# lbcb-sci/herro

Hardware: AMD Instinct MI355X
Metric: 4096-bp windows corrected/sec at batch=128 (higher is better)
Workload: dtype f16; 1 GPU; synthetic windows, 4096 bp, 32 overlaps each, batch=128, 1xMI355X per rank (BASELINE configs[2]); batch=128, window=4096, overlaps=32, batches_per_launch_group=32, streams_per_gpu=2, distinct_windows_cycled=16384, precision=5, total_windows=165760, strong_leg_windows=0

## Files before the change

herro_amd/csrc/pileup.hip:

```cpp
#include <hip/hip_runtime.h>
#include <stdint.h>

#include <cstdio>
#include <cstdlib>
#include <mutex>
#include <set>
#include <type_traits>

#include "job_dev.h"
#include "pileup_core.h"

namespace herro {

namespace {

constexpr uint32_t NONE = 0xffffffffu;
constexpr uint32_t RF_LEFT = 0x80000000u;
constexpr uint32_t ROWCAP = HERRO_TILE;
constexpr uint32_t SCAP = 128;
constexpr uint32_t QEVCAP = 2048;

template <int NT>
__device__ __forceinline__ uint32_t blk_scan(uint32_t v, uint32_t* total, uint32_t* s_wave ) {
  const int lane = threadIdx.x & 63, wave = threadIdx.x >> 6;
// ... 484 lines not shown
  PROF_MARK(J, 1, 2);
  const bool in_lds = n <= RKCAP;
  if (in_lds)
    for (uint32_t i = tid; i < n; i += NT) { s_acc[i] = J.ow_acc[wd.ow_begin + i]; s_keep[i] = J.ow_keep[wd.ow_begin + i]; }
  __syncthreads();
  if (tid < 32 && tid < n && ((keepmask >> tid) & 1u) && s_ns) {
    const uint32_t cls = ocol[wd.ow_begin + tid].w, nm = (s_nm2[tid & 15u] >> (tid & 16u)) & 0xffffu, ns = s_ns;
    if (nm) atomicAdd(&J.nd[2 * (uint64_t)cls], nm);
    if (ns - nm) atomicAdd(&J.nd[2 * (uint64_t)cls + 1], ns - nm);
  }
  auto rank_all = [&](auto lds) {
    constexpr bool LDS = decltype(lds)::value;
    for (uint32_t i = tid; i < n; i += NT) {
      const uint32_t oi = wd.ow_begin + i;
      const uint32_t ki = LDS ? (uint32_t)s_keep[i] : (uint32_t)J.ow_keep[oi];
      if (!ki) continue;
      const float ai = LDS ? s_acc[i] : J.ow_acc[oi];
      uint32_t rank = 0;
      for (uint32_t j = 0; j < n; j++) {
        const uint32_t kj = LDS ? (uint32_t)s_keep[j] : (uint32_t)J.ow_keep[wd.ow_begin + j];
        const float aj = LDS ? s_acc[j] : J.ow_acc[wd.ow_begin + j];
        if (kj && (aj > ai || (aj == ai && j < i))) rank++;
      }
      J.slot_ow[wd.ow_begin + rank] = oi;
    }
  };
  if (in_lds) rank_all(std::true_type{}); else rank_all(std::false_type{});
  if (tid == 0) J.win_nkept[w] = n_kept;
  PROF_MARK(J, 1, 3);
}

constexpr int LY_NT = 256;
constexpr uint32_t TCAP = 2 * LY_NT;
#define MI(p) ((p) + ((p) >> 4))
__host__ __device__ inline size_t layout_lds(uint32_t W) { return (size_t)(W + 1 + ((W + 1) >> 4) + 1) * 4; }

template <bool TILES>
__global__ __launch_bounds__(LY_NT) void k_layout(JobDev J) {
  extern __shared__ __attribute__((aligned(16))) uint32_t ly_smem[];
  uint32_t* s_mi = ly_smem;
  __shared__ double s_score[SCAP];
  __shared__ uint32_t s_sel[32], s_nev[32], s_evoff[32], s_wave[LY_NT / 64], s_maxne, s_nrun;
  __shared__ uint32_t s_tcnt[TCAP], s_toff[TCAP];
  const uint32_t w = blockIdx.x, tid = threadIdx.x;
  PROF_BEGIN(J);
  const WinDesc wd = J.win[w];
  const uint32_t n_kept = J.win_nkept[w];
  const uint32_t win_len = wd.win_len;
  if (tid < 32) s_sel[tid] = NONE;
  if (tid == 0) { s_maxne = 0; s_nrun = 0; }
  if constexpr (TILES) for (uint32_t t = tid; t < TCAP; t += LY_NT) s_tcnt[t] = 0;
  for (uint32_t p = tid; p <= win_len; p += LY_NT) s_mi[MI(p)] = 0;
  __syncthreads();
  PROF_MARK(J, 2, 5);
  {
    auto score_of = [&](uint32_t k) -> double {
      const uint32_t cls = J.ocol[J.slot_ow[wd.ow_begin + k]].w;
      const uint32_t nn = J.nd[2 * (uint64_t)cls], dd = J.nd[2 * (uint64_t)cls + 1];
      const uint32_t tot = nn + dd;
      if (!tot) return 0.0;
      const double lg = tot < J.ln_table_n ? J.ln_table[tot] : log((double)tot + 1.0);
      return __dmul_rn(__ddiv_rn((double)nn, (double)tot), lg);
    };
    const bool cached = n_kept <= SCAP;
    if (cached) {
      for (uint32_t k = tid; k < n_kept; k += LY_NT) s_score[k] = score_of(k);
      __syncthreads();
      PROF_MARK(J, 2, 6);
    }
    for (uint32_t k = tid; k < n_kept; k += LY_NT) {
      const uint32_t o = J.slot_ow[wd.ow_begin + k];
      const uint32_t qid = J.ow[o].qid;
      const double sk = cached ? s_score[k] : score_of(k);
      uint32_t rank = 0;
      if (cached) {
        uint32_t i = 0;
        for (; i + 8 <= n_kept; i += 8) {
          double sv[8];
#pragma unroll
          for (int u = 0; u < 8; u++) sv[u] = s_score[i + u];
#pragma unroll
          for (int u = 0; u < 8; u++) if (sv[u] > sk || (sv[u] == sk && i + u < k)) rank++;
        }
        for (; i < n_kept; i++) {
          const double si = s_score[i];
          if (si > sk || (si == sk && i < k)) rank++;
        }
      } else {
        for (uint32_t i = 0; i < n_kept; i++) {
          const double si = score_of(i);
          if (si > sk || (si == sk && i < k)) rank++;
        }
      }
      J.rank_qid[wd.ow_begin + rank] = qid;
      if (rank < 30u) s_sel[rank + 1] = o;
    }
    __syncthreads();
  }
  PROF_MARK(J, 2, 0);
  if (tid < 32) {
    CTab t;
    t.off = 0; t.t_total = 0; t.tokc = (uint32_t)TOK_GAP_F << 8; t.ow = NONE; t.n_ev = 0; t.ev_off = 0; t.sbase = 0; t.sdir = 1;
    t.qual_off = 0; t.q_woff = 0;
    if (tid == 0) {
      t.t_total = win_len;
      t.q_woff = J.read_word_off[wd.rid];
      t.qual_off = J.read_qual_off[wd.rid];
    } else if (s_sel[tid] != NONE) {
      const uint32_t o = s_sel[tid];
      const OwDesc& d = J.ow[o];
      t.off = (int32_t)(d.tstart - d.wtstart);
      t.t_total = J.ow_ttotal[o];
      t.tokc = d.strand ? (5u | ((uint32_t)TOK_GAP_R << 8)) : ((uint32_t)TOK_GAP_F << 8);
      t.ow = o;
      t.n_ev = J.ins_cnt[o];
      t.ev_off = d.scr_off;
      t.sbase = d.strand ? (int32_t)(d.qbeg + d.qlen - 1u) : (int32_t)d.qbeg;
      t.sdir = d.strand ? -1 : 1;
      t.qual_off = d.q_qual_off;
      t.q_woff = d.q_woff;
    }
    const uint32_t nev = tid == 0 ? 0u : t.n_ev;
    const uint32_t inc = wscan_incl(nev);
    const uint32_t tot = (uint32_t)__builtin_amdgcn_readlane((int)inc, 31);
    if (tid == 0) {
      t.ev_off = (uint32_t)wd.ev_off;
      t.n_ev = tot;
    }
    J.ctab[(uint64_t)w * 32 + tid] = t;
    J.sel_ow[(uint64_t)w * 32 + tid] = s_sel[tid];
    s_nev[tid] = nev;
    s_evoff[tid] = tid == 0 ? 0u : t.ev_off;
    if (tid == 0) s_evoff[0] = t.ev_off;
    atomicMax(&s_maxne, nev);
  }
  __syncthreads();
  PROF_MARK(J, 2, 1);
  const uint32_t lc = tid >> 3, sub = tid & 7u;
  const uint32_t ne = s_nev[lc];
  const uint64_t eo = s_evoff[lc], wbase = s_evoff[0];
  const uint32_t nbatch = (s_maxne + 63u) / 64u;
  uint4 v[8];
  uint32_t hx[8];
  auto load = [&](uint32_t b) {
#pragma unroll
    for (int k = 0; k < 8; k++) {
      const uint32_t i = b * 64u + sub + 8u * k;
      v[k] = ne ? J.iev[eo + min(i, ne - 1u)] : make_uint4(0, 0, 0, 0);
      if constexpr (TILES) hx[k] = ne ? J.iev[eo + min(i + 1u, ne - 1u)].x : 0u; else hx[k] = 0u;
    }
  };
  for (uint32_t b = 0; b < nbatch; b++) {
    load(b);
#pragma unroll
    for (int k = 0; k < 8; k++) {
      const uint32_t i = b * 64u + sub + 8u * k;
      if (i < ne) {
        const uint32_t p = v[k].x & 0xffffu;
        if (p < win_len) atomicMax(&s_mi[MI(p)], v[k].w);
      }
    }
  }
  __syncthreads();
  PROF_MARK(J, 2, 2);
  {
    const uint32_t ch = (win_len + LY_NT - 1) / LY_NT;
    const uint32_t p0 = min(tid * ch, win_len), p1 = min(p0 + ch, win_len);
    uint32_t local = 0;
    for (uint32_t p = p0; p < p1; p++) local += 1u + s_mi[MI(p)];
    uint32_t Lf;
    uint32_t r = blk_scan<LY_NT>(local, &Lf, s_wave);
    const uint32_t tile0 = (uint32_t)wd.col_off;
    for (uint32_t p = p0; p < p1; p++) {
      const uint32_t rn = r + 1u + s_mi[MI(p)];
      s_mi[MI(p)] = r;
      const uint32_t i = (rn - 1u) / ROWCAP;
      if (i * ROWCAP >= r) J.chdr2[tile0 + i] = make_uint2(p, r == i * ROWCAP ? 1u : 0u);
      r = rn;
    }
    if (tid == 0) { s_mi[MI(win_len)] = Lf; J.win_Lf[w] = Lf; }
  }
  __syncthreads();
  PROF_MARK(J, 2, 3);
  for (uint32_t p = tid; p <= win_len; p += LY_NT) J.row_of_pos2[wd.pos_off + p] = s_mi[MI(p)];
  const uint32_t tile0 = (uint32_t)wd.col_off, n_t = (s_mi[MI(win_len)] + ROWCAP - 1) / ROWCAP;
  auto each_run = [&](uint32_t b, auto&& fn) {
    if (nbatch > 1) load(b);
#pragma unroll
    for (int k = 0; k < 8; k++) {
      const uint32_t i = b * 64u + sub + 8u * k;
      if (i >= ne) continue;
      const uint32_t p = v[k].x & 0xffffu, len = v[k].x >> 16;
      if (p >= win_len) continue;
      const uint32_t rp = s_mi[MI(p)], room = s_mi[MI(p + 1)] - rp - 1u;
      uint32_t hide = 0;
      if (i + 1 < ne && (hx[k] & 0xffffu) == p) {
        hide = hx[k] >> 16;
        for (uint32_t e2 = i + 2; e2 < ne; e2++) {
          const uint32_t x3 = J.iev[eo + e2].x;
          if ((x3 & 0xffffu) != p) break;
          hide = max(hide, x3 >> 16);
        }
      }
      const uint32_t lenr = min(len, room);
      if (hide >= lenr) continue;
      fn(v[k], hide, (rp + 1u + hide) / ROWCAP, (rp + lenr) / ROWCAP);
    }
  };
  if constexpr (!TILES) {
    (void)n_t; (void)tile0; (void)wbase; (void)each_run;
  } else {
  for (uint32_t b = 0; b < nbatch; b++)
    each_run(b, [&](const uint4&, uint32_t, uint32_t t_lo, uint32_t t_hi) {
      for (uint32_t t = t_lo; t <= t_hi && t < TCAP; t++) atomicAdd(&s_tcnt[t], 1u);
    });
  __syncthreads();
  {
    uint32_t tot;
    const uint32_t c0 = s_tcnt[2 * tid], c1 = s_tcnt[2 * tid + 1];
    const uint32_t ex = blk_scan<LY_NT>(c0 + c1, &tot, s_wave);
    s_toff[2 * tid] = ex;
    s_toff[2 * tid + 1] = ex + c0;
    if (2 * tid < n_t) J.tile_ev[tile0 + 2 * tid] = make_uint2(ex, c0);
    if (2 * tid + 1 < n_t) J.tile_ev[tile0 + 2 * tid + 1] = make_uint2(ex + c0, c1);
  }
  __syncthreads();
  for (uint32_t b = 0; b < nbatch; b++)
    each_run(b, [&](const uint4& e, uint32_t hide, uint32_t t_lo, uint32_t t_hi) {
      for (uint32_t t = t_lo; t <= t_hi && t < TCAP; t++)
        J.tev[wbase + atomicAdd(&s_toff[t], 1u)] = make_uint4(e.x, e.y, e.z, lc | (hide << 8) | (t << 16));
    });
  }
  PROF_MARK(J, 2, 4);
}

constexpr int TK_NT = 256;
constexpr uint32_t WPAD = 36;

__device__ __forceinline__ uint32_t dpp_quad_add(uint32_t v) {
  v += (uint32_t)__builtin_amdgcn_mov_dpp((int)v, 0xB1, 0xf, 0xf, true);
  v += (uint32_t)__builtin_amdgcn_mov_dpp((int)v, 0x4E, 0xf, 0xf, true);
  return v;
}
__device__ __forceinline__ uint32_t dpp_quad_lane0(uint32_t v) {
  return (uint32_t)__builtin_amdgcn_mov_dpp((int)v, 0x00, 0xf, 0xf, true);
}

__global__ __launch_bounds__(TK_NT, 4) void k_tokens(JobDev J, uint32_t aux) {
  __shared__ __attribute__((aligned(16))) CTab s_ct[32];
  __shared__ __attribute__((aligned(16))) uint16_t s_rowinfo[ROWCAP];
  __shared__ uint32_t s_adj[ROWCAP];
  __shared__ uint32_t s_pl[HERRO_ROWS * 3 * WPAD];
  __shared__ uint32_t s_rop[ROWCAP + 4];
  __shared__ uint32_t s_supbits[ROWCAP / 32];
  const uint32_t tile = blockIdx.x, tid = threadIdx.x, nw = J.nw;
  PROF_BEGIN(J);
  const uint32_t w = J.tile_win[tile], r0 = J.tile_r0[tile];
  const uint32_t Lf = J.win_Lf[w];
  if (r0 >= Lf) return;
  const WinDesc wd = J.win[w];
  const uint2 ch0 = J.chdr2[tile];
  const bool last = r0 + ROWCAP >= Lf;
  const uint2 ch1 = J.chdr2[last ? tile : tile + 1];
  const uint2 tev_h = J.tile_ev[tile];
  if (tid < 32) s_ct[tid] = J.ctab[(uint64_t)w * 32 + tid];
// ... 227 lines not shown
  PROF_MARK(J, 3, 6);
}

__global__ __launch_bounds__(64) void k_supgather(JobDev J) {
  const uint32_t w = blockIdx.x, lane = threadIdx.x;
  const WinDesc wd = J.win[w];
  const uint32_t Lf = J.win_Lf[w], tile0 = (uint32_t)wd.col_off;
  const uint32_t nch = (Lf + ROWCAP - 1) / ROWCAP;
  uint32_t dst = 0;
  for (uint32_t c0 = 0; c0 < nch; c0 += 64) {
    const uint32_t i = c0 + lane;
    const uint32_t cn = i < nch ? J.tile_nsup[tile0 + i] : 0u;
    const uint32_t inc = wscan_incl(cn);
    const uint32_t my_dst = dst + inc - cn;
    for (uint32_t j = 0; j < 64 && c0 + j < nch; j++) {
      const uint32_t cnt_j = (uint32_t)__builtin_amdgcn_readlane((int)cn, (int)j), dst_j = (uint32_t)__builtin_amdgcn_readlane((int)my_dst, (int)j);
      const uint32_t src = (c0 + j) * ROWCAP;
      if (src == dst_j) continue;
      for (uint32_t k = lane; k < cnt_j; k += 64) {
        const uint32_t a = J.sup_row[wd.row_off + src + k], b = J.sup_pi[wd.row_off + src + k];
        J.sup_row[wd.row_off + dst_j + k] = a;
        J.sup_pi[wd.row_off + dst_j + k] = b;
      }
    }
    dst += wlast(inc);
  }
  if (lane == 0) J.win_nsup[w] = dst;
}

#ifndef HERRO_RW_ICAP
#define HERRO_RW_ICAP 2048
#endif
constexpr uint32_t RW_ICAP = HERRO_RW_ICAP;
#define RI(p) ((p) + ((p) >> 5))
__host__ __device__ inline size_t rows_lds(uint32_t W) { return (size_t)(W + 2 + ((W + 2) >> 5) + 1) * 4; }

constexpr uint32_t RW_SUPCAP = 256;
template <int SP>
__device__ __forceinline__ void rf_slot(const JobDev& J, const CTab* __restrict__ s_ct, const WinDesc& wd, uint32_t Lf, uint32_t half, uint32_t c,
                                        uint32_t srow, uint32_t pj, uint32_t nr, bool have_nr, uint4* __restrict__ out);

template <int NW>
__global__ __launch_bounds__(2 * NW) void k_rows(JobDev J) {
  constexpr int NT = 2 * NW;
  extern __shared__ __attribute__((aligned(16))) uint32_t rw_smem[];
  uint32_t* s_rop = rw_smem;
  uint32_t* s_mrg = rw_smem + rows_lds(J.window_size) / 4;
  __shared__ __attribute__((aligned(16))) CTab s_ct[32];
  __shared__ uint32_t s_adj[RW_ICAP];
  __shared__ __attribute__((aligned(16))) uint8_t s_iv[RW_ICAP];
  __shared__ uint32_t s_rfbase;
  __shared__ uint32_t s_sup[3][RW_SUPCAP];
  __shared__ uint32_t s_wave[NT / 64];
  const uint32_t w = blockIdx.x, tid = threadIdx.x, nw = J.nw;
  const uint32_t half = tid >= (uint32_t)NW ? 1u : 0u, lt = tid - half * NW;
  PROF_BEGIN(J);
  const WinDesc wd = J.win[w];
  const uint32_t Lf = J.win_Lf[w], win_len = wd.win_len;
  const uint32_t tile0 = (uint32_t)wd.col_off;
  {
    constexpr int RL = 17;
    uint32_t rv[RL];
    const uint32_t* __restrict__ rop = J.row_of_pos2 + wd.pos_off;
#pragma unroll
    for (int u = 0; u < RL; u++) rv[u] = rop[min(tid + (uint32_t)u * NT, win_len)];
    if (tid < 32) s_ct[tid] = J.ctab[(uint64_t)w * 32 + tid];
#pragma unroll
    for (int u = 0; u < RL; u++) {
      const uint32_t p = tid + (uint32_t)u * NT;
      if (p <= win_len) s_rop[RI(p)] = rv[u];
    }
  }
  __syncthreads();
  PROF_MARK(J, 6, 0);
  const bool active = lt < nw;
  const uint32_t widx = min(lt, nw - 1u);
  const int32_t P = (int32_t)(widx << 5);
  const uint32_t vm = active ? mask_range(0, (int32_t)win_len - P) : 0u;
  const uint64_t pmax = J.read_n_words + 1;
  const uint32_t tlo = glb_bits(J.read_p0, s_ct[0].q_woff, pmax, (int32_t)wd.tstart + P) & vm;
  const uint32_t thi = glb_bits(J.read_p1, s_ct[0].q_woff, pmax, (int32_t)wd.tstart + P) & vm;
  uint32_t c0[5], c1[5];
  uint32_t nin[5];
  const uint32_t tsym[4] = {vm & ~tlo & ~thi, tlo & ~thi, thi & ~tlo, tlo & thi};
#pragma unroll
  for (int q = 0; q < 4; q++) { c0[q] = half ? 0u : tsym[q]; c1[q] = 0; }
  c0[4] = 0; c1[4] = 0;
  nin[0] = half ? 0u : vm; nin[1] = 0; nin[2] = 0; nin[3] = 0; nin[4] = 0;
  auto sat_add = [&](int q, uint32_t x) { sat2_add(c0[q], c1[q], x); };
  {
    constexpr int UB = 15;
    const uint32_t cb = 1u + UB * half;
    uint32_t M[UB], L[UB], H[UB];
#pragma unroll
    for (int u = 0; u < UB; u++) {
      const uint32_t o = s_ct[cb + u].ow;
      const PlaneRec g = J.cw[(o != NONE ? (uint64_t)o : 0ull) * nw + widx];
      M[u] = g.m; L[u] = g.lo; H[u] = g.hi;
    }
    PROF_MARK(J, 6, 10);
#pragma unroll
    for (int u = 0; u < UB; u++) {
      const CTab& h = s_ct[cb + u];
      const uint32_t tt = h.ow != NONE ? h.t_total : 0u;
      const uint32_t inr = mask_range(h.off - P, h.off + (int32_t)tt - P) & vm;
      const uint32_t Mi = M[u] & inr, Li = L[u] & Mi, Hi = H[u] & Mi;
      sat_add(0, Mi & ~Li & ~Hi);
      sat_add(1, Li & ~Hi);
      sat_add(2, Hi & ~Li);
      sat_add(3, Li & Hi);
      sat_add(4, inr & ~Mi);
      uint32_t x = inr;
#pragma unroll
      for (int b = 0; b < 5; b++) { const uint32_t cy = nin[b] & x; nin[b] ^= x; x = cy; }
    }
  }
  if (half) {
#pragma unroll
    for (int q = 0; q < 5; q++) { s_mrg[(q) * NW + lt] = c0[q]; s_mrg[(5 + q) * NW + lt] = c1[q]; s_mrg[(10 + q) * NW + lt] = nin[q]; }
  }
  __syncthreads();
  if (!half) {
#pragma unroll
    for (int q = 0; q < 5; q++) sat2_merge(c0[q], c1[q], s_mrg[q * NW + lt], s_mrg[(5 + q) * NW + lt]);
    uint32_t cy = 0;
#pragma unroll
    for (int b = 0; b < 5; b++) {
      const uint32_t x = nin[b], y = s_mrg[(10 + b) * NW + lt];
      nin[b] = x ^ y ^ cy;
      cy = (x & y) | (cy & (x ^ y));
    }
  }
  const bool lane0 = !half && active;
  constexpr uint32_t IP_ROWS = (RW_ICAP * 2 + NW * 4 - 1) / (NW * 4);
  static_assert(IP_ROWS + 7 <= 15, "s_mrg holds the insertion rows' positions, five cover planes and two words per lane");
  uint16_t* s_ip = reinterpret_cast<uint16_t*>(s_mrg);
  uint32_t* s_nin = s_mrg + IP_ROWS * NW;
  uint32_t* s_insup = s_nin + 5 * NW;
  uint32_t* s_nisup = s_insup + NW;
  if (!half) {
#pragma unroll
    for (int b = 0; b < 5; b++) s_nin[b * NW + lt] = nin[b];
    s_insup[lt] = 0;
    s_nisup[lt] = 0;
  }
  PROF_MARK(J, 6, 1);
  const RowVotes rvt = base_row_votes(c0, c1, tsym, vm);
  const uint32_t supb = lane0 ? rvt.sup : 0u, V0 = rvt.v0, V1 = rvt.v1, V2 = rvt.v2;
  uint32_t insmask = 0;
  if (lane0) {
    uint32_t rprev = s_rop[RI((uint32_t)P)];
#pragma unroll 4
    for (uint32_t k = 0; k < 32; k++) {
      const uint32_t p = (uint32_t)P + k;
      const uint32_t rn = s_rop[RI(min(p + 1u, win_len))];
      if (p < win_len && rn - rprev > 1u) insmask |= 1u << k;
      rprev = rn;
    }
    uint32_t* __restrict__ vp = J.vpl + (uint64_t)w * 4 * nw + lt;
    vp[0] = V0; vp[nw] = V1; vp[2 * nw] = V2; vp[3 * nw] = insmask;
  }
  PROF_MARK(J, 6, 2);
  const uint32_t n_irows = Lf - win_len;
  uint32_t n_isup = 0, insup = 0;
  for (uint32_t ch0 = 0; ch0 < n_irows; ch0 += RW_ICAP) {
    if (ch0) __syncthreads();
    for (uint32_t i = tid; i < min(RW_ICAP, n_irows - ch0); i += NT) s_adj[i] = 0;
    __syncthreads();
    PROF_MARK(J, 6, 7);
    constexpr uint32_t TPC = NT / 32;
    constexpr int EU = 6;
    const uint32_t c = tid / TPC, sub = tid % TPC;
    const uint32_t ne = (c >= 1u && s_ct[c].ow != NONE) ? s_ct[c].n_ev : 0u;
    const uint4* __restrict__ iev = J.iev + s_ct[c].ev_off;
    for (uint32_t i0 = sub; i0 < ne; i0 += EU * TPC) {
      uint4 ve[EU];
      uint32_t nx[EU];
#pragma unroll
      for (int u = 0; u < EU; u++) {
        const uint32_t i = i0 + u * TPC;
        ve[u] = iev[min(i, ne - 1u)];
        nx[u] = iev[min(i + 1u, ne - 1u)].x;
      }
#pragma unroll
      for (int u = 0; u < EU; u++) {
        const uint32_t i = i0 + u * TPC;
        if (i >= ne) continue;
        const uint32_t p = ve[u].x & 0xffffu, len = ve[u].x >> 16;
        if (p >= win_len) continue;
        const uint32_t rp = s_rop[RI(p)], room = s_rop[RI(p + 1)] - rp - 1u;
        uint32_t hide = 0;
        if (i + 1u < ne && (nx[u] & 0xffffu) == p) {
          hide = nx[u] >> 16;
          for (uint32_t e2 = i + 2u; e2 < ne; e2++) {
            const uint32_t x3 = iev[e2].x;
            if ((x3 & 0xffffu) != p) break;
            hide = max(hide, x3 >> 16);
          }
        }
        const bool inr = (uint32_t)((int32_t)p - s_ct[c].off) < s_ct[c].t_total;
        for (uint32_t k = hide; k < len && k < room; k++) {
          const uint32_t ir = rp + k - p - ch0;
          if (ir >= RW_ICAP) continue;
          uint32_t code;
          if (k < 16u) code = ((ve[u].z >> k) & 1u) | (((ve[u].z >> (16u + k)) & 1u) << 1);
          else {
            const int32_t si = s_ct[c].sbase + s_ct[c].sdir * (int32_t)(ve[u].y + k);
            const uint64_t wi = min(s_ct[c].q_woff + ((uint32_t)si >> 5), pmax);
            code = ((J.read_p0[wi] >> ((uint32_t)si & 31u)) & 1u) | (((J.read_p1[wi] >> ((uint32_t)si & 31u)) & 1u) << 1);
            if (s_ct[c].sdir < 0) code ^= 3u;
          }
          atomicAdd(&s_adj[ir], (1u << (5u * code)) + (inr ? 1u << 20 : 0u));
          s_ip[ir] = (uint16_t)p;
        }
      }
    }
    __syncthreads();
    PROF_MARK(J, 6, 8);
    for (uint32_t i = tid; i < min(RW_ICAP, n_irows - ch0); i += NT) {
      const uint32_t adj = s_adj[i];
      uint32_t cover = 0, p = 0;
      if (adj) {
        p = s_ip[i];
        const uint32_t pw = p >> 5, pb = p & 31u;
        cover = ((s_nin[pw] >> pb) & 1u) | (((s_nin[NW + pw] >> pb) & 1u) << 1) | (((s_nin[2 * NW + pw] >> pb) & 1u) << 2) |
                (((s_nin[3 * NW + pw] >> pb) & 1u) << 3) | (((s_nin[4 * NW + pw] >> pb) & 1u) << 4);
      }
      const uint32_t c5[5] = {adj & 31u, (adj >> 5) & 31u, (adj >> 10) & 31u, (adj >> 15) & 31u, cover - (adj >> 20)};
      uint32_t ns = 0;
#pragma unroll
      for (int q = 0; q < 5; q++) ns += c5[q] >= 3u ? 1u : 0u;
      s_iv[i] = (uint8_t)(vote5(c5, 4u) | ((ns >= 2u ? 1u : 0u) << 7));
      if (ns >= 2u) { atomicOr(&s_insup[p >> 5], 1u << (p & 31u)); atomicAdd(&s_nisup[p >> 5], 1u); }
    }
    __syncthreads();
    PROF_MARK(J, 6, 9);
    if (lane0) { insup = s_insup[lt]; n_isup = s_nisup[lt]; }
    {
      const uint32_t nb = min(RW_ICAP, n_irows - ch0);
      uint32_t* __restrict__ dst = reinterpret_cast<uint32_t*>(J.cons_tmp + wd.row_off + ch0);
      for (uint32_t i = tid; i * 4u < nb; i += NT) dst[i] = reinterpret_cast<const uint32_t*>(s_iv)[i];
    }
  }
// ... 695 lines not shown
  KT_BEGIN(tm, "rf_quals", st);
  if (rf && 2 * half + 1 <= 8) {
    if (half <= 2u) hipLaunchKernelGGL(k_rfq<5>, dim3(J.n_win), dim3(RQ_NT), 0, st, J, half, sup_off, rf, cap, (lean ? 1u : 0u) | (left_only ? 2u : 0u));
    else hipLaunchKernelGGL(k_rfq<8>, dim3(J.n_win), dim3(RQ_NT), 0, st, J, half, sup_off, rf, cap, (lean ? 1u : 0u) | (left_only ? 2u : 0u));
    KT_END(tm, st);
    return;
  }
  pileup_opt_in_lds(reinterpret_cast<const void*>(k_quals<false>), 96 * 1024);
  hipLaunchKernelGGL(k_quals<false>, dim3(J.n_win), dim3(PQ_NT), quals_lds(J.nw), st, J, half);
  KT_END(tm, st);
}

void launch_full_quals(const JobDev& J, hipStream_t st) {
  if (!J.n_win) return;
  pileup_opt_in_lds(reinterpret_cast<const void*>(k_quals<true>), 96 * 1024);
  hipLaunchKernelGGL(k_quals<true>, dim3(J.n_win), dim3(PQ_NT), quals_lds(J.nw), st, J, 0u);
}

template <int NB>
static void launch_win(const JobDev& J, hipStream_t st) {
  hipLaunchKernelGGL(k_win<NB>, dim3(J.n_win), dim3(J.nw <= 128 ? 128 : 256), 0, st, J);
}

static void trace_point(const char* name, hipStream_t st) {
  static const bool on = [] { const char* e = getenv("HERRO_TRACE"); return e && atoi(e); }();
  if (!on) return;
  const hipError_t e = hipStreamSynchronize(st);
  fprintf(stderr, "TRACE %s done: %s\n", name, hipGetErrorString(e));
}

void launch_full_tokens(const JobDev& J, hipStream_t st, KernelTimer* tm) {
  if (!J.n_win || !J.n_tiles) return;
  KT_BEGIN(tm, "tokens", st);
  hipLaunchKernelGGL(k_layout<true>, dim3(J.n_win), dim3(LY_NT), layout_lds(J.window_size), st, J);
  hipLaunchKernelGGL(k_tokens, dim3(J.n_tiles), dim3(TK_NT), 0, st, J, 0u);
  KT_END(tm, st);
  trace_point("tokens (planes on request)", st);
}

void launch_featurize(const JobDev& J, hipStream_t st, KernelTimer* tm, bool lean) {
  if (!J.n_win) return;
  if (J.n_ow) {
    KT_BEGIN(tm, "cols", st);
    if (J.nw <= 128) hipLaunchKernelGGL((k_cols<3, 2>), dim3((J.n_ow + CA_NW - 1) / CA_NW), dim3(CA_NT), (size_t)CA_NW * cols_lds_words(J.nw) * 4, st, J);
    else hipLaunchKernelGGL((k_cols<5, 4>), dim3((J.n_ow + CA_NW - 1) / CA_NW), dim3(CA_NT), (size_t)CA_NW * cols_lds_words(J.nw) * 4, st, J);
    KT_END(tm, st);
  trace_point("cols", st);
  }
  KT_BEGIN(tm, "win", st);
  if (J.n_cls) (void)hipMemsetAsync(J.nd, 0, (size_t)J.n_cls * 8, st);
  {
    const uint32_t tmax = (uint32_t)((double)(J.max_cols > 31 ? J.max_cols : 31) * 0.1);
    if (tmax < 4) launch_win<2>(J, st);
    else if (tmax < 8) launch_win<3>(J, st);
    else if (tmax < 16) launch_win<4>(J, st);
    else if (tmax < 64) launch_win<6>(J, st);
    else if (tmax < 512) launch_win<9>(J, st);
    else launch_win<14>(J, st);
  }
  KT_END(tm, st);
  trace_point("win", st);
  KT_BEGIN(tm, "layout", st);
  if (lean) hipLaunchKernelGGL(k_layout<false>, dim3(J.n_win), dim3(LY_NT), layout_lds(J.window_size), st, J);
  else hipLaunchKernelGGL(k_layout<true>, dim3(J.n_win), dim3(LY_NT), layout_lds(J.window_size), st, J);
  KT_END(tm, st);
  trace_point("layout", st);
  if (lean) {
    KT_BEGIN(tm, "rows", st);
    if (J.nw <= 128) {
      pileup_opt_in_lds(reinterpret_cast<const void*>(k_rows<128>), 96 * 1024);
      hipLaunchKernelGGL(k_rows<128>, dim3(J.n_win), dim3(256), rows_lds(J.window_size) + (size_t)15 * 128 * 4, st, J);
    } else {
      pileup_opt_in_lds(reinterpret_cast<const void*>(k_rows<256>), 96 * 1024);
      hipLaunchKernelGGL(k_rows<256>, dim3(J.n_win), dim3(512), rows_lds(J.window_size) + (size_t)15 * 256 * 4, st, J);
    }
    KT_END(tm, st);
    trace_point("rows", st);
    return;
  }
  KT_BEGIN(tm, "tokens", st);
  if (J.n_tiles) hipLaunchKernelGGL(k_tokens, dim3(J.n_tiles), dim3(TK_NT), 0, st, J, 1u);
  KT_END(tm, st);
  trace_point("tokens", st);
  KT_BEGIN(tm, "supgather", st);
  hipLaunchKernelGGL(k_supgather, dim3(J.n_win), dim3(64), 0, st, J);
  KT_END(tm, st);
  trace_point("supgather", st);
}

}
```

Before: 3.478 million windows/s.

## Fuse layout scoring, ranking and insertion scan into the rows kernel on the lean path

On the lean path, the separate k_layout launch is removed and its work (score and rank of kept overlaps, column table build, max-insertion scan, row-of-position prefix) moves into k_rows. The aim is to drop one kernel launch plus the global round-trip of ctab, win_Lf and row_of_pos2 between kernels. k_rows also derives the insertion mask from a bitmask built during the scan, prefetches plane records earlier to overlap the layout work, and gets a min-blocks launch bound. The cost is more LDS and register pressure in k_rows and duplicated layout logic shared through helpers.

```diff
diff --git a/herro_amd/csrc/pileup.hip b/herro_amd/csrc/pileup.hip
--- a/herro_amd/csrc/pileup.hip
+++ b/herro_amd/csrc/pileup.hip
@@ -540,15 +540,173 @@
 
 constexpr int LY_NT = 256;
 constexpr uint32_t TCAP = 2 * LY_NT;
-#define MI(p) ((p) + ((p) >> 4))
-__host__ __device__ inline size_t layout_lds(uint32_t W) { return (size_t)(W + 1 + ((W + 1) >> 4) + 1) * 4; }
-
-template <bool TILES>
+#define RI(p) ((p) + ((p) >> 5))
+__host__ __device__ inline size_t rows_lds(uint32_t W) { return (((size_t)(W + 2 + ((W + 2) >> 5) + 1) * 4) + 7) & ~(size_t)7; }
+
+__device__ __forceinline__ double layout_score(const JobDev& J, const WinDesc& wd, uint32_t k) {
+  const uint32_t cls = J.ocol[J.slot_ow[wd.ow_begin + k]].w;
+  const uint32_t nn = J.nd[2 * (uint64_t)cls], dd = J.nd[2 * (uint64_t)cls + 1];
+  const uint32_t tot = nn + dd;
+  if (!tot) return 0.0;
+  const double lg = tot < J.ln_table_n ? J.ln_table[tot] : log((double)tot + 1.0);
+  return __dmul_rn(__ddiv_rn((double)nn, (double)tot), lg);
+}
+struct LayoutCol { uint32_t o, qid; CTab t; };
+__device__ __forceinline__ LayoutCol layout_col(const JobDev& J, const WinDesc& wd, uint32_t k) {
+  LayoutCol c;
+  const uint32_t o = J.slot_ow[wd.ow_begin + k];
+  const OwDesc& d = J.ow[o];
+  c.o = o;
+  c.qid = d.qid;
+  c.t.off = (int32_t)(d.tstart - d.wtstart);
+  c.t.t_total = J.ow_ttotal[o];
+  c.t.tokc = d.strand ? (5u | ((uint32_t)TOK_GAP_R << 8)) : ((uint32_t)TOK_GAP_F << 8);
+  c.t.ow = o;
+  c.t.n_ev = J.ins_cnt[o];
+  c.t.ev_off = d.scr_off;
+  c.t.sbase = d.strand ? (int32_t)(d.qbeg + d.qlen - 1u) : (int32_t)d.qbeg;
+  c.t.sdir = d.strand ? -1 : 1;
+  c.t.qual_off = d.q_qual_off;
+  c.t.q_woff = d.q_woff;
+  return c;
+}
+template <int NT>
+__device__ __forceinline__ LayoutCol layout_scores(const JobDev& J, const WinDesc& wd, uint32_t n_kept, double* __restrict__ s_score) {
+  static_assert(SCAP <= (uint32_t)NT, "one kept overlap per thread where the scores are cached");
+  LayoutCol c = {};
+  if (n_kept <= SCAP && threadIdx.x < n_kept) {
+    c = layout_col(J, wd, threadIdx.x);
+    s_score[threadIdx.x] = layout_score(J, wd, threadIdx.x);
+  }
+  return c;
+}
+template <int NT>
+__device__ __forceinline__ void layout_rank(const JobDev& J, const WinDesc& wd, uint32_t n_kept, const double* __restrict__ s_score, const LayoutCol& pre,
+                                            uint32_t* __restrict__ s_sel, CTab* __restrict__ s_ct) {
+  const bool cached = n_kept <= SCAP;
+  for (uint32_t k = threadIdx.x; k < n_kept; k += NT) {
+    const LayoutCol c = cached ? pre : layout_col(J, wd, k);
+    const double sk = cached ? s_score[k] : layout_score(J, wd, k);
+    uint32_t rank = 0;
+    if (cached) {
+      uint32_t i = 0;
+      for (; i + 8 <= n_kept; i += 8) {
+        double sv[8];
+#pragma unroll
+        for (int u = 0; u < 8; u++) sv[u] = s_score[i + u];
+#pragma unroll
+        for (int u = 0; u < 8; u++) if (sv[u] > sk || (sv[u] == sk && i + u < k)) rank++;
+      }
+      for (; i < n_kept; i++) {
+        const double si = s_score[i];
+        if (si > sk || (si == sk && i < k)) rank++;
+      }
+    } else {
+      for (uint32_t i = 0; i < n_kept; i++) {
+        const double si = layout_score(J, wd, i);
+        if (si > sk || (si == sk && i < k)) rank++;
+      }
+    }
+    J.rank_qid[wd.ow_begin + rank] = c.qid;
+    if (rank < 30u) { s_sel[rank + 1] = c.o; s_ct[rank + 1] = c.t; }
+  }
+}
+__device__ __forceinline__ CTab layout_ctab(const JobDev& J, uint32_t w, const WinDesc& wd, const uint32_t* __restrict__ s_sel, CTab* __restrict__ s_ct,
+                                            uint64_t t_woff, uint64_t t_qoff) {
+  const uint32_t tid = threadIdx.x;
+  CTab t;
+  t.off = 0; t.t_total = 0; t.tokc = (uint32_t)TOK_GAP_F << 8; t.ow = NONE; t.n_ev = 0; t.ev_off = 0; t.sbase = 0; t.sdir = 1;
+  t.qual_off = 0; t.q_woff = 0;
+  if (tid == 0) {
+    t.t_total = wd.win_len;
+    t.q_woff = t_woff;
+    t.qual_off = t_qoff;
+  } else if (s_sel[tid] != NONE) {
+    t = s_ct[tid];
+  }
+  const uint32_t inc = wscan_incl(tid == 0 ? 0u : t.n_ev);
+  const uint32_t tot = (uint32_t)__builtin_amdgcn_readlane((int)inc, 31);
+  if (tid == 0) {
+    t.ev_off = (uint32_t)wd.ev_off;
+    t.n_ev = tot;
+  }
+  s_ct[tid] = t;
+  J.ctab[(uint64_t)w * 32 + tid] = t;
+  J.sel_ow[(uint64_t)w * 32 + tid] = s_sel[tid];
+  return t;
+}
+template <int TPC>
+struct EvBatch {
+  uint4 v[8];
+  uint32_t hx[8];
+  __device__ __forceinline__ static uint32_t index(uint32_t b, uint32_t sub, int k) { return b * (8u * TPC) + sub + (uint32_t)TPC * k; }
+  __device__ __forceinline__ void load(const uint4* __restrict__ iev, uint32_t ne, uint32_t b, uint32_t sub) {
+#pragma unroll
+    for (int k = 0; k < 8; k++) {
+      const uint32_t i = index(b, sub, k);
+      v[k] = ne ? iev[min(i, ne - 1u)] : make_uint4(0, 0, 0, 0);
+      hx[k] = ne ? iev[min(i + 1u, ne - 1u)].x : 0u;
+    }
+  }
+  __device__ __forceinline__ void max_ins(uint32_t ne, uint32_t b, uint32_t sub, uint32_t win_len, uint32_t* __restrict__ s_mi) const {
+#pragma unroll
+    for (int k = 0; k < 8; k++) {
+      if (index(b, sub, k) < ne) {
+        const uint32_t p = v[k].x & 0xffffu;
+        if (p < win_len) atomicMax(&s_mi[RI(p)], v[k].w);
+      }
+    }
+  }
+  __device__ __forceinline__ uint32_t hidden(const uint4* __restrict__ iev, uint32_t ne, uint32_t i, int k, uint32_t p) const {
+    uint32_t hide = 0;
+    if (i + 1u < ne && (hx[k] & 0xffffu) == p) {
+      hide = hx[k] >> 16;
+      for (uint32_t e2 = i + 2u; e2 < ne; e2++) {
+        const uint32_t x3 = iev[e2].x;
+        if ((x3 & 0xffffu) != p) break;
+        hide = max(hide, x3 >> 16);
+      }
+    }
+    return hide;
+  }
+};
+template <int NT, bool CHDR>
+__device__ __forceinline__ uint32_t layout_scan(const JobDev& J, uint32_t w, const WinDesc& wd, uint32_t* __restrict__ s_mi, uint32_t* s_wave, uint32_t* __restrict__ s_im = nullptr) {
+  const uint32_t tid = threadIdx.x, win_len = wd.win_len;
+  const uint32_t ch = (win_len + NT - 1) / NT;
+  const uint32_t p0 = min(tid * ch, win_len), p1 = min(p0 + ch, win_len);
+  uint32_t local = 0, im = 0;
+  for (uint32_t p = p0; p < p1; p++) {
+    const uint32_t mi = s_mi[RI(p)];
+    local += 1u + mi;
+    if (s_im) {
+      if ((p & 31u) == 0u && im) { atomicOr(&s_im[(p >> 5) - 1u], im); im = 0; }
+      if (mi) im |= 1u << (p & 31u);
+    }
+  }
+  if (s_im && im) atomicOr(&s_im[(p1 - 1u) >> 5], im);
+  uint32_t Lf;
+  uint32_t r = blk_scan<NT>(local, &Lf, s_wave);
+  const uint32_t tile0 = (uint32_t)wd.col_off;
+  for (uint32_t p = p0; p < p1; p++) {
+    const uint32_t rn = r + 1u + s_mi[RI(p)];
+    s_mi[RI(p)] = r;
+    if constexpr (CHDR) {
+      const uint32_t i = (rn - 1u) / ROWCAP;
+      if (i * ROWCAP >= r) J.chdr2[tile0 + i] = make_uint2(p, r == i * ROWCAP ? 1u : 0u);
+    }
+    r = rn;
+  }
+  if (tid == 0) { s_mi[RI(win_len)] = Lf; J.win_Lf[w] = Lf; }
+  return Lf;
+}
+
 __global__ __launch_bounds__(LY_NT) void k_layout(JobDev J) {
   extern __shared__ __attribute__((aligned(16))) uint32_t ly_smem[];
   uint32_t* s_mi = ly_smem;
   __shared__ double s_score[SCAP];
-  __shared__ uint32_t s_sel[32], s_nev[32], s_evoff[32], s_wave[LY_NT / 64], s_maxne, s_nrun;
+  __shared__ __attribute__((aligned(16))) CTab s_ct[32];
+  __shared__ uint32_t s_sel[32], s_nev[32], s_evoff[32], s_wave[LY_NT / 64], s_maxne;
   __shared__ uint32_t s_tcnt[TCAP], s_toff[TCAP];
   const uint32_t w = blockIdx.x, tid = threadIdx.x;
   PROF_BEGIN(J);
@@ -556,168 +714,61 @@
   const uint32_t n_kept = J.win_nkept[w];
   const uint32_t win_len = wd.win_len;
   if (tid < 32) s_sel[tid] = NONE;
-  if (tid == 0) { s_maxne = 0; s_nrun = 0; }
-  if constexpr (TILES) for (uint32_t t = tid; t < TCAP; t += LY_NT) s_tcnt[t] = 0;
-  for (uint32_t p = tid; p <= win_len; p += LY_NT) s_mi[MI(p)] = 0;
+  if (tid == 0) s_maxne = 0;
+  for (uint32_t t = tid; t < TCAP; t += LY_NT) s_tcnt[t] = 0;
+  for (uint32_t p = tid; p <= win_len; p += LY_NT) s_mi[RI(p)] = 0;
   __syncthreads();
   PROF_MARK(J, 2, 5);
-  {
-    auto score_of = [&](uint32_t k) -> double {
-      const uint32_t cls = J.ocol[J.slot_ow[wd.ow_begin + k]].w;
-      const uint32_t nn = J.nd[2 * (uint64_t)cls], dd = J.nd[2 * (uint64_t)cls + 1];
-      const uint32_t tot = nn + dd;
-      if (!tot) return 0.0;
-      const double lg = tot < J.ln_table_n ? J.ln_table[tot] : log((double)tot + 1.0);
-      return __dmul_rn(__ddiv_rn((double)nn, (double)tot), lg);
-    };
-    const bool cached = n_kept <= SCAP;
-    if (cached) {
-      for (uint32_t k = tid; k < n_kept; k += LY_NT) s_score[k] = score_of(k);
-      __syncthreads();
-      PROF_MARK(J, 2, 6);
-    }
-    for (uint32_t k = tid; k < n_kept; k += LY_NT) {
-      const uint32_t o = J.slot_ow[wd.ow_begin + k];
-      const uint32_t qid = J.ow[o].qid;
-      const double sk = cached ? s_score[k] : score_of(k);
-      uint32_t rank = 0;
-      if (cached) {
-        uint32_t i = 0;
-        for (; i + 8 <= n_kept; i += 8) {
-          double sv[8];
-#pragma unroll
-          for (int u = 0; u < 8; u++) sv[u] = s_score[i + u];
-#pragma unroll
-          for (int u = 0; u < 8; u++) if (sv[u] > sk || (sv[u] == sk && i + u < k)) rank++;
-        }
-        for (; i < n_kept; i++) {
-          const double si = s_score[i];
-          if (si > sk || (si == sk && i < k)) rank++;
-        }
-      } else {
-        for (uint32_t i = 0; i < n_kept; i++) {
-          const double si = score_of(i);
-          if (si > sk || (si == sk && i < k)) rank++;
-        }
-      }
-      J.rank_qid[wd.ow_begin + rank] = qid;
-      if (rank < 30u) s_sel[rank + 1] = o;
-    }
+  const LayoutCol pre = layout_scores<LY_NT>(J, wd, n_kept, s_score);
+  if (n_kept <= SCAP) {
     __syncthreads();
-  }
+    PROF_MARK(J, 2, 6);
+  }
+  const uint64_t t_woff = J.read_word_off[wd.rid], t_qoff = J.read_qual_off[wd.rid];
+  layout_rank<LY_NT>(J, wd, n_kept, s_score, pre, s_sel, s_ct);
+  __syncthreads();
   PROF_MARK(J, 2, 0);
   if (tid < 32) {
-    CTab t;
-    t.off = 0; t.t_total = 0; t.tokc = (uint32_t)TOK_GAP_F << 8; t.ow = NONE; t.n_ev = 0; t.ev_off = 0; t.sbase = 0; t.sdir = 1;
-    t.qual_off = 0; t.q_woff = 0;
-    if (tid == 0) {
-      t.t_total = win_len;
-      t.q_woff = J.read_word_off[wd.rid];
-      t.qual_off = J.read_qual_off[wd.rid];
-    } else if (s_sel[tid] != NONE) {
-      const uint32_t o = s_sel[tid];
-      const OwDesc& d = J.ow[o];
-      t.off = (int32_t)(d.tstart - d.wtstart);
-      t.t_total = J.ow_ttotal[o];
-      t.tokc = d.strand ? (5u | ((uint32_t)TOK_GAP_R << 8)) : ((uint32_t)TOK_GAP_F << 8);
-      t.ow = o;
-      t.n_ev = J.ins_cnt[o];
-      t.ev_off = d.scr_off;
-      t.sbase = d.strand ? (int32_t)(d.qbeg + d.qlen - 1u) : (int32_t)d.qbeg;
-      t.sdir = d.strand ? -1 : 1;
-      t.qual_off = d.q_qual_off;
-      t.q_woff = d.q_woff;
-    }
-    const uint32_t nev = tid == 0 ? 0u : t.n_ev;
-    const uint32_t inc = wscan_incl(nev);
-    const uint32_t tot = (uint32_t)__builtin_amdgcn_readlane((int)inc, 31);
-    if (tid == 0) {
-      t.ev_off = (uint32_t)wd.ev_off;
-      t.n_ev = tot;
-    }
-    J.ctab[(uint64_t)w * 32 + tid] = t;
-    J.sel_ow[(uint64_t)w * 32 + tid] = s_sel[tid];
-    s_nev[tid] = nev;
-    s_evoff[tid] = tid == 0 ? 0u : t.ev_off;
-    if (tid == 0) s_evoff[0] = t.ev_off;
-    atomicMax(&s_maxne, nev);
+    const CTab t = layout_ctab(J, w, wd, s_sel, s_ct, t_woff, t_qoff);
+    s_nev[tid] = tid == 0 ? 0u : t.n_ev;
+    s_evoff[tid] = t.ev_off;
+    atomicMax(&s_maxne, s_nev[tid]);
   }
   __syncthreads();
   PROF_MARK(J, 2, 1);
-  const uint32_t lc = tid >> 3, sub = tid & 7u;
+  constexpr int TPC = LY_NT / 32;
+  const uint32_t lc = tid / TPC, sub = tid % TPC;
   const uint32_t ne = s_nev[lc];
-  const uint64_t eo = s_evoff[lc], wbase = s_evoff[0];
-  const uint32_t nbatch = (s_maxne + 63u) / 64u;
-  uint4 v[8];
-  uint32_t hx[8];
-  auto load = [&](uint32_t b) {
+  const uint4* __restrict__ iev = J.iev + (lc ? s_evoff[lc] : 0u);
+  const uint64_t wbase = s_evoff[0];
+  const uint32_t nbatch = (s_maxne + 8u * TPC - 1u) / (8u * TPC);
+  EvBatch<TPC> ev;
+  for (uint32_t b = 0; b < nbatch; b++) {
+    ev.load(iev, ne, b, sub);
+    ev.max_ins(ne, b, sub, win_len, s_mi);
+  }
+  __syncthreads();
+  PROF_MARK(J, 2, 2);
+  const uint32_t Lf = layout_scan<LY_NT, true>(J, w, wd, s_mi, s_wave);
+  __syncthreads();
+  PROF_MARK(J, 2, 3);
+  for (uint32_t p = tid; p <= win_len; p += LY_NT) J.row_of_pos2[wd.pos_off + p] = s_mi[RI(p)];
+  const uint32_t tile0 = (uint32_t)wd.col_off, n_t = (Lf + ROWCAP - 1) / ROWCAP;
+  auto each_run = [&](uint32_t b, auto&& fn) {
+    if (nbatch > 1) ev.load(iev, ne, b, sub);
 #pragma unroll
     for (int k = 0; k < 8; k++) {
-      const uint32_t i = b * 64u + sub + 8u * k;
-      v[k] = ne ? J.iev[eo + min(i, ne - 1u)] : make_uint4(0, 0, 0, 0);
-      if constexpr (TILES) hx[k] = ne ? J.iev[eo + min(i + 1u, ne - 1u)].x : 0u; else hx[k] = 0u;
-    }
-  };
-  for (uint32_t b = 0; b < nbatch; b++) {
-    load(b);
-#pragma unroll
-    for (int k = 0; k < 8; k++) {
-      const uint32_t i = b * 64u + sub + 8u * k;
-      if (i < ne) {
-        const uint32_t p = v[k].x & 0xffffu;
-        if (p < win_len) atomicMax(&s_mi[MI(p)], v[k].w);
-      }
-    }
-  }
-  __syncthreads();
-  PROF_MARK(J, 2, 2);
-  {
-    const uint32_t ch = (win_len + LY_NT - 1) / LY_NT;
-    const uint32_t p0 = min(tid * ch, win_len), p1 = min(p0 + ch, win_len);
-    uint32_t local = 0;
-    for (uint32_t p = p0; p < p1; p++) local += 1u + s_mi[MI(p)];
-    uint32_t Lf;
-    uint32_t r = blk_scan<LY_NT>(local, &Lf, s_wave);
-    const uint32_t tile0 = (uint32_t)wd.col_off;
-    for (uint32_t p = p0; p < p1; p++) {
-      const uint32_t rn = r + 1u + s_mi[MI(p)];
-      s_mi[MI(p)] = r;
-      const uint32_t i = (rn - 1u) / ROWCAP;
-      if (i * ROWCAP >= r) J.chdr2[tile0 + i] = make_uint2(p, r == i * ROWCAP ? 1u : 0u);
-      r = rn;
-    }
-    if (tid == 0) { s_mi[MI(win_len)] = Lf; J.win_Lf[w] = Lf; }
-  }
-  __syncthreads();
-  PROF_MARK(J, 2, 3);
-  for (uint32_t p = tid; p <= win_len; p += LY_NT) J.row_of_pos2[wd.pos_off + p] = s_mi[MI(p)];
-  const uint32_t tile0 = (uint32_t)wd.col_off, n_t = (s_mi[MI(win_len)] + ROWCAP - 1) / ROWCAP;
-  auto each_run = [&](uint32_t b, auto&& fn) {
-    if (nbatch > 1) load(b);
-#pragma unroll
-    for (int k = 0; k < 8; k++) {
-      const uint32_t i = b * 64u + sub + 8u * k;
+      const uint32_t i = EvBatch<TPC>::index(b, sub, k);
       if (i >= ne) continue;
-      const uint32_t p = v[k].x & 0xffffu, len = v[k].x >> 16;
+      const uint32_t p = ev.v[k].x & 0xffffu, len = ev.v[k].x >> 16;
       if (p >= win_len) continue;
-      const uint32_t rp = s_mi[MI(p)], room = s_mi[MI(p + 1)] - rp - 1u;
-      uint32_t hide = 0;
-      if (i + 1 < ne && (hx[k] & 0xffffu) == p) {
-        hide = hx[k] >> 16;
-        for (uint32_t e2 = i + 2; e2 < ne; e2++) {
-          const uint32_t x3 = J.iev[eo + e2].x;
-          if ((x3 & 0xffffu) != p) break;
-          hide = max(hide, x3 >> 16);
-        }
-      }
+      const uint32_t rp = s_mi[RI(p)], room = s_mi[RI(p + 1)] - rp - 1u;
+      const uint32_t hide = ev.hidden(iev, ne, i, k, p);
       const uint32_t lenr = min(len, room);
       if (hide >= lenr) continue;
-      fn(v[k], hide, (rp + 1u + hide) / ROWCAP, (rp + lenr) / ROWCAP);
+      fn(ev.v[k], hide, (rp + 1u + hide) / ROWCAP, (rp + lenr) / ROWCAP);
     }
   };
-  if constexpr (!TILES) {
-    (void)n_t; (void)tile0; (void)wbase; (void)each_run;
-  } else {
   for (uint32_t b = 0; b < nbatch; b++)
     each_run(b, [&](const uint4&, uint32_t, uint32_t t_lo, uint32_t t_hi) {
       for (uint32_t t = t_lo; t <= t_hi && t < TCAP; t++) atomicAdd(&s_tcnt[t], 1u);
@@ -738,7 +789,6 @@
       for (uint32_t t = t_lo; t <= t_hi && t < TCAP; t++)
         J.tev[wbase + atomicAdd(&s_toff[t], 1u)] = make_uint4(e.x, e.y, e.z, lc | (hide << 8) | (t << 16));
     });
-  }
   PROF_MARK(J, 2, 4);
 }
 
@@ -1032,16 +1082,13 @@
 #define HERRO_RW_ICAP 2048
 #endif
 constexpr uint32_t RW_ICAP = HERRO_RW_ICAP;
-#define RI(p) ((p) + ((p) >> 5))
-__host__ __device__ inline size_t rows_lds(uint32_t W) { return (size_t)(W + 2 + ((W + 2) >> 5) + 1) * 4; }
-
 constexpr uint32_t RW_SUPCAP = 256;
 template <int SP>
 __device__ __forceinline__ void rf_slot(const JobDev& J, const CTab* __restrict__ s_ct, const WinDesc& wd, uint32_t Lf, uint32_t half, uint32_t c,
                                         uint32_t srow, uint32_t pj, uint32_t nr, bool have_nr, uint4* __restrict__ out);
 
 template <int NW>
-__global__ __launch_bounds__(2 * NW) void k_rows(JobDev J) {
+__global__ __launch_bounds__(2 * NW, 4) void k_rows(JobDev J) {
   constexpr int NT = 2 * NW;
   extern __shared__ __attribute__((aligned(16))) uint32_t rw_smem[];
   uint32_t* s_rop = rw_smem;
@@ -1051,35 +1098,58 @@
   __shared__ __attribute__((aligned(16))) uint8_t s_iv[RW_ICAP];
   __shared__ uint32_t s_rfbase;
   __shared__ uint32_t s_sup[3][RW_SUPCAP];
-  __shared__ uint32_t s_wave[NT / 64];
+  __shared__ uint32_t s_wave[NT / 64], s_maxne;
   const uint32_t w = blockIdx.x, tid = threadIdx.x, nw = J.nw;
   const uint32_t half = tid >= (uint32_t)NW ? 1u : 0u, lt = tid - half * NW;
   PROF_BEGIN(J);
   const WinDesc wd = J.win[w];
-  const uint32_t Lf = J.win_Lf[w], win_len = wd.win_len;
-  const uint32_t tile0 = (uint32_t)wd.col_off;
-  {
-    constexpr int RL = 17;
-    uint32_t rv[RL];
-    const uint32_t* __restrict__ rop = J.row_of_pos2 + wd.pos_off;
-#pragma unroll
-    for (int u = 0; u < RL; u++) rv[u] = rop[min(tid + (uint32_t)u * NT, win_len)];
-    if (tid < 32) s_ct[tid] = J.ctab[(uint64_t)w * 32 + tid];
-#pragma unroll
-    for (int u = 0; u < RL; u++) {
-      const uint32_t p = tid + (uint32_t)u * NT;
-      if (p <= win_len) s_rop[RI(p)] = rv[u];
-    }
-  }
-  __syncthreads();
-  PROF_MARK(J, 6, 0);
+  const uint32_t n_kept = J.win_nkept[w], win_len = wd.win_len;
+  double* s_score = reinterpret_cast<double*>(s_mrg);
+  uint32_t* s_sel = s_sup[0];
+  uint32_t* s_im = s_sup[1];
+  static_assert((uint32_t)NW <= RW_SUPCAP, "s_im borrows a row of s_sup");
+  if (tid < 32) s_sel[tid] = NONE;
+  if (tid < (uint32_t)NW) s_im[tid] = 0;
+  if (tid == 0) s_maxne = 0;
+  for (uint32_t p = tid; p <= win_len; p += NT) s_rop[RI(p)] = 0;
   const bool active = lt < nw;
   const uint32_t widx = min(lt, nw - 1u);
   const int32_t P = (int32_t)(widx << 5);
   const uint32_t vm = active ? mask_range(0, (int32_t)win_len - P) : 0u;
   const uint64_t pmax = J.read_n_words + 1;
-  const uint32_t tlo = glb_bits(J.read_p0, s_ct[0].q_woff, pmax, (int32_t)wd.tstart + P) & vm;
-  const uint32_t thi = glb_bits(J.read_p1, s_ct[0].q_woff, pmax, (int32_t)wd.tstart + P) & vm;
+  __syncthreads();
+  PROF_MARK(J, 6, 0);
+  const uint64_t t_woff = J.read_word_off[wd.rid], t_qoff = J.read_qual_off[wd.rid];
+  const LayoutCol pre = layout_scores<NT>(J, wd, n_kept, s_score);
+  if (n_kept <= SCAP) __syncthreads();
+  const uint64_t tw0 = min(t_woff + (((uint32_t)wd.tstart + (uint32_t)P) >> 5), pmax), tw1 = min(t_woff + (((uint32_t)wd.tstart + (uint32_t)P) >> 5) + 1, pmax);
+  const uint32_t tl0 = J.read_p0[tw0], tl1 = J.read_p0[tw1], th0 = J.read_p1[tw0], th1 = J.read_p1[tw1];
+  layout_rank<NT>(J, wd, n_kept, s_score, pre, s_sel, s_ct);
+  __syncthreads();
+  PROF_MARK(J, 6, 11);
+  if (tid < 32) {
+    const CTab t = layout_ctab(J, w, wd, s_sel, s_ct, t_woff, t_qoff);
+    atomicMax(&s_maxne, tid == 0 ? 0u : t.n_ev);
+  }
+  __syncthreads();
+  PROF_MARK(J, 6, 12);
+  constexpr int TPC = NT / 32;
+  const uint32_t ec = tid / TPC, sub = tid % TPC;
+  const uint32_t ne = (ec >= 1u && s_ct[ec].ow != NONE) ? s_ct[ec].n_ev : 0u;
+  const uint4* __restrict__ iev = J.iev + (ec ? s_ct[ec].ev_off : 0u);
+  const uint32_t nbatch = (s_maxne + 8u * TPC - 1u) / (8u * TPC);
+  constexpr int UB = 15;
+  const uint32_t cb = 1u + UB * half;
+  uint32_t M[UB], L[UB], H[UB];
+#pragma unroll
+  for (int u = 0; u < UB; u++) {
+    const uint32_t o = s_ct[cb + u].ow;
+    const PlaneRec g = J.cw[(o != NONE ? (uint64_t)o : 0ull) * nw + widx];
+    M[u] = g.m; L[u] = g.lo; H[u] = g.hi;
+  }
+  const uint32_t ev_touch = ne ? iev[min(8u * sub, ne - 1u)].x : 0u;
+  const uint32_t tlo = __funnelshift_r(tl0, tl1, ((uint32_t)wd.tstart + (uint32_t)P) & 31u) & vm;
+  const uint32_t thi = __funnelshift_r(th0, th1, ((uint32_t)wd.tstart + (uint32_t)P) & 31u) & vm;
   uint32_t c0[5], c1[5];
   uint32_t nin[5];
   const uint32_t tsym[4] = {vm & ~tlo & ~thi, tlo & ~thi, thi & ~tlo, tlo & thi};
@@ -1089,15 +1159,6 @@
   nin[0] = half ? 0u : vm; nin[1] = 0; nin[2] = 0; nin[3] = 0; nin[4] = 0;
   auto sat_add = [&](int q, uint32_t x) { sat2_add(c0[q], c1[q], x); };
   {
-    constexpr int UB = 15;
-    const uint32_t cb = 1u + UB * half;
-    uint32_t M[UB], L[UB], H[UB];
-#pragma unroll
-    for (int u = 0; u < UB; u++) {
-      const uint32_t o = s_ct[cb + u].ow;
-      const PlaneRec g = J.cw[(o != NONE ? (uint64_t)o : 0ull) * nw + widx];
-      M[u] = g.m; L[u] = g.lo; H[u] = g.hi;
-    }
     PROF_MARK(J, 6, 10);
 #pragma unroll
     for (int u = 0; u < UB; u++) {
@@ -1147,20 +1208,26 @@
   PROF_MARK(J, 6, 1);
   const RowVotes rvt = base_row_votes(c0, c1, tsym, vm);
   const uint32_t supb = lane0 ? rvt.sup : 0u, V0 = rvt.v0, V1 = rvt.v1, V2 = rvt.v2;
+  PROF_MARK(J, 6, 2);
+  asm volatile("" :: "v"(ev_touch));
+  EvBatch<TPC> ev;
+  for (uint32_t b = 0; b < nbatch; b++) {
+    ev.load(iev, ne, b, sub);
+    ev.max_ins(ne, b, sub, win_len, s_rop);
+  }
+  __syncthreads();
+  PROF_MARK(J, 6, 13);
+  const uint32_t Lf = layout_scan<NT, false>(J, w, wd, s_rop, s_wave, s_im);
+  __syncthreads();
+  PROF_MARK(J, 6, 14);
+  for (uint32_t p = tid; p <= win_len; p += NT) J.row_of_pos2[wd.pos_off + p] = s_rop[RI(p)];
   uint32_t insmask = 0;
   if (lane0) {
-    uint32_t rprev = s_rop[RI((uint32_t)P)];
-#pragma unroll 4
-    for (uint32_t k = 0; k < 32; k++) {
-      const uint32_t p = (uint32_t)P + k;
-      const uint32_t rn = s_rop[RI(min(p + 1u, win_len))];
-      if (p < win_len && rn - rprev > 1u) insmask |= 1u << k;
-      rprev = rn;
-    }
+    insmask = s_im[lt] & vm;
     uint32_t* __restrict__ vp = J.vpl + (uint64_t)w * 4 * nw + lt;
     vp[0] = V0; vp[nw] = V1; vp[2 * nw] = V2; vp[3 * nw] = insmask;
   }
-  PROF_MARK(J, 6, 2);
+  PROF_MARK(J, 6, 6);
   const uint32_t n_irows = Lf - win_len;
   uint32_t n_isup = 0, insup = 0;
   for (uint32_t ch0 = 0; ch0 < n_irows; ch0 += RW_ICAP) {
@@ -1168,47 +1235,28 @@
     for (uint32_t i = tid; i < min(RW_ICAP, n_irows - ch0); i += NT) s_adj[i] = 0;
     __syncthreads();
     PROF_MARK(J, 6, 7);
-    constexpr uint32_t TPC = NT / 32;
-    constexpr int EU = 6;
-    const uint32_t c = tid / TPC, sub = tid % TPC;
-    const uint32_t ne = (c >= 1u && s_ct[c].ow != NONE) ? s_ct[c].n_ev : 0u;
-    const uint4* __restrict__ iev = J.iev + s_ct[c].ev_off;
-    for (uint32_t i0 = sub; i0 < ne; i0 += EU * TPC) {
-      uint4 ve[EU];
-      uint32_t nx[EU];
-#pragma unroll
-      for (int u = 0; u < EU; u++) {
-        const uint32_t i = i0 + u * TPC;
-        ve[u] = iev[min(i, ne - 1u)];
-        nx[u] = iev[min(i + 1u, ne - 1u)].x;
-      }
-#pragma unroll
-      for (int u = 0; u < EU; u++) {
-        const uint32_t i = i0 + u * TPC;
+    for (uint32_t b = 0; b < nbatch; b++) {
+      if (nbatch > 1u) ev.load(iev, ne, b, sub);
+#pragma unroll
+      for (int u = 0; u < 8; u++) {
+        const uint32_t i = EvBatch<TPC>::index(b, sub, u);
         if (i >= ne) continue;
-        const uint32_t p = ve[u].x & 0xffffu, len = ve[u].x >> 16;
+        const uint4 ve = ev.v[u];
+        const uint32_t p = ve.x & 0xffffu, len = ve.x >> 16;
         if (p >= win_len) continue;
         const uint32_t rp = s_rop[RI(p)], room = s_rop[RI(p + 1)] - rp - 1u;
-        uint32_t hide = 0;
-        if (i + 1u < ne && (nx[u] & 0xffffu) == p) {
-          hide = nx[u] >> 16;
-          for (uint32_t e2 = i + 2u; e2 < ne; e2++) {
-            const uint32_t x3 = iev[e2].x;
-            if ((x3 & 0xffffu) != p) break;
-            hide = max(hide, x3 >> 16);
-          }
-        }
-        const bool inr = (uint32_t)((int32_t)p - s_ct[c].off) < s_ct[c].t_total;
+        const uint32_t hide = ev.hidden(iev, ne, i, u, p);
+        const bool inr = (uint32_t)((int32_t)p - s_ct[ec].off) < s_ct[ec].t_total;
         for (uint32_t k = hide; k < len && k < room; k++) {
           const uint32_t ir = rp + k - p - ch0;
           if (ir >= RW_ICAP) continue;
           uint32_t code;
-          if (k < 16u) code = ((ve[u].z >> k) & 1u) | (((ve[u].z >> (16u + k)) & 1u) << 1);
+          if (k < 16u) code = ((ve.z >> k) & 1u) | (((ve.z >> (16u + k)) & 1u) << 1);
           else {
-            const int32_t si = s_ct[c].sbase + s_ct[c].sdir * (int32_t)(ve[u].y + k);
-            const uint64_t wi = min(s_ct[c].q_woff + ((uint32_t)si >> 5), pmax);
+            const int32_t si = s_ct[ec].sbase + s_ct[ec].sdir * (int32_t)(ve.y + k);
+            const uint64_t wi = min(s_ct[ec].q_woff + ((uint32_t)si >> 5), pmax);
             code = ((J.read_p0[wi] >> ((uint32_t)si & 31u)) & 1u) | (((J.read_p1[wi] >> ((uint32_t)si & 31u)) & 1u) << 1);
-            if (s_ct[c].sdir < 0) code ^= 3u;
+            if (s_ct[ec].sdir < 0) code ^= 3u;
           }
           atomicAdd(&s_adj[ir], (1u << (5u * code)) + (inr ? 1u << 20 : 0u));
           s_ip[ir] = (uint16_t)p;
@@ -1970,7 +2018,7 @@
 void launch_full_tokens(const JobDev& J, hipStream_t st, KernelTimer* tm) {
   if (!J.n_win || !J.n_tiles) return;
   KT_BEGIN(tm, "tokens", st);
-  hipLaunchKernelGGL(k_layout<true>, dim3(J.n_win), dim3(LY_NT), layout_lds(J.window_size), st, J);
+  hipLaunchKernelGGL(k_layout, dim3(J.n_win), dim3(LY_NT), rows_lds(J.window_size), st, J);
   hipLaunchKernelGGL(k_tokens, dim3(J.n_tiles), dim3(TK_NT), 0, st, J, 0u);
   KT_END(tm, st);
   trace_point("tokens (planes on request)", st);
@@ -1998,11 +2046,6 @@
   }
   KT_END(tm, st);
   trace_point("win", st);
-  KT_BEGIN(tm, "layout", st);
-  if (lean) hipLaunchKernelGGL(k_layout<false>, dim3(J.n_win), dim3(LY_NT), layout_lds(J.window_size), st, J);
-  else hipLaunchKernelGGL(k_layout<true>, dim3(J.n_win), dim3(LY_NT), layout_lds(J.window_size), st, J);
-  KT_END(tm, st);
-  trace_point("layout", st);
   if (lean) {
     KT_BEGIN(tm, "rows", st);
     if (J.nw <= 128) {
@@ -2016,6 +2059,10 @@
     trace_point("rows", st);
     return;
   }
+  KT_BEGIN(tm, "layout", st);
+  hipLaunchKernelGGL(k_layout, dim3(J.n_win), dim3(LY_NT), rows_lds(J.window_size), st, J);
+  KT_END(tm, st);
+  trace_point("layout", st);
   KT_BEGIN(tm, "tokens", st);
   if (J.n_tiles) hipLaunchKernelGGL(k_tokens, dim3(J.n_tiles), dim3(TK_NT), 0, st, J, 1u);
   KT_END(tm, st);
```

Result: faster. 3.521 million windows/s, median of 6 (+1.3%).
